# ethz-asl/multipoint

Hardware: AMD Instinct MI355X
Metric: image-pairs/sec (detect+desc+match) @ 480x640 (higher is better)
Workload: dtype f32

## Files before the change

multipoint_amd/build.py:

```python
import concurrent.futures
import os
import subprocess
import sys

HERE = os.path.dirname(os.path.abspath(__file__))
CSRC = os.path.join(HERE, 'csrc')
OBJ_DIR = os.path.join(CSRC, '_build')
LIB_PATH = os.path.join(HERE, 'libmultipoint_hip.so')
SOURCES = ['conv_mfma.hip', 'conv_wino43.hip', 'conv_wino43b.hip', 'conv_split.hip', 'conv_f16.hip', 'conv_f16_res.hip', 'conv_first.hip', 'heads_post.hip', 'head_tail.hip', 'head_tail_f16.hip', 'nms.hip', 'keypoints.hip',
           'sample_desc.hip', 'match_mfma.hip', 'match_guided.hip', 'match_extra.hip', 'pair_metrics.hip', 'detector_metrics.hip', 'homography.hip', 'homography_pooled.hip', 'homog_adapt.hip', 'losses.hip', 'batchnorm_stats.hip', 'photometric.hip', 'shapes.hip', 'api.hip',
           'model_load.hip', 'forward.hip', 'post_api.hip', 'mutual_info.hip', 'align_api.hip', 'pyramid.hip', 'fft.hip', 'lghd.hip', 'lghd_api.hip', 'frames.hip',
           'frames_api.hip', 'draw.hip']
HEADERS = [os.path.join(CSRC, h) for h in ('mp_common.h', 'mp_device.h', 'mp_tile.h', 'mp_f16.h', 'mp_match.h', 'mp_fft.h', 'mp_raster.h', 'mp_homography.h', 'mp_f16_store_pooled.inc',
                                            'mp_f16_store_lines.inc', 'host.h')] + [
    os.path.join(HERE, '..', 'include', 'multipoint_hip.h')]
HIPCC = os.environ.get('HIPCC', '/opt/rocm/bin/hipcc')
FLAGS = ['--offload-arch=gfx950', '-O3', '-std=c++17', '-fPIC', '-Wall', '-Wno-unused-function'] + \
    os.environ.get('MP_HIPCC_FLAGS', '').split()


def _stale(target, deps):
    if not os.path.exists(target):
        return True
    t = os.path.getmtime(target)
    return any(os.path.getmtime(d) > t for d in deps)


DMA_SOURCES = ('conv_wino43.hip', 'conv_wino43b.hip', 'head_tail.hip', 'head_tail_f16.hip')


def check_dma_hazards(asm_path, wait_states=5):
    import re
    lines = open(asm_path).read().split('\n')
    n = 0
    for i, l in enumerate(lines):
        m = re.search(r'global_load_lds_dword(?:x4)? v\d+, s\[(\d+):(\d+)\]', l)
        if not m:
            continue
        n += 1
        base = {int(m.group(1)), int(m.group(2))}
        ws, j = 0, i - 1
        while j >= 0 and ws < wait_states:
            t = lines[j].strip()
            j -= 1
            if t.endswith(':') and not t.startswith(('.Lfunc', ';')) and re.match(r'\.LBB\d+_\d+:', t):
                raise RuntimeError('%s:%d: LDS-DMA only %d wait states behind the branch target %s (needs %d inside the '
                                   'block): open the asm statement with s_nop' % (asm_path, j + 2, ws, t, wait_states))
            if not t or t.startswith((';', '.')) or t.endswith(':'):
                continue
            w = re.match(r'(v_readlane_b32|v_readfirstlane_b32) s(\d+),', t)
            if w and int(w.group(2)) in base:
                raise RuntimeError('%s:%d: %s writes the base SGPR of an LDS-DMA only %d wait states later (needs %d): '
                                   'open the asm statement with s_nop' % (asm_path, j + 2, t, ws, wait_states))
            nop = re.match(r's_nop (\d+)', t)
            ws += int(nop.group(1)) + 1 if nop else 1
    if n == 0:
        raise RuntimeError('%s: no global_load_lds found -- the hazard check is looking at the wrong file' % asm_path)
    return n


SCRATCH_CAPS = {'conv_mfma.hip': 0, 'conv_wino43.hip': 0, 'conv_wino43b.hip': 136, 'conv_split.hip': 0, 'conv_f16.hip': 12,
                'conv_f16_res.hip': 0, 'conv_first.hip': 0, 'head_tail.hip': 0, 'head_tail_f16.hip': 0, 'losses.hip': 0,
                'batchnorm_stats.hip': 0, 'photometric.hip': 0, 'shapes.hip': 0, 'match_mfma.hip': 0, 'match_guided.hip': 0, 'mutual_info.hip': 0, 'pyramid.hip': 0, 'fft.hip': 0, 'lghd.hip': 0,
                'frames.hip': 0, 'draw.hip': 0}


def check_scratch(asm_path, cap):
    import re
    text = open(asm_path).read()
    found = re.findall(r'\.name:\s+(\S+)\n(?:(?!\.name:).*\n)*?\s+\.private_segment_fixed_size:\s+(\d+)', text)
    if not found:
        raise RuntimeError('%s: no kernel metadata found -- the scratch check is looking at the wrong file' % asm_path)
    used = {k: int(v) for k, v in found if int(v) > 0}
    over = {k: v for k, v in used.items() if v > cap}
    if over:
        raise RuntimeError('%s: %d kernel(s) use more scratch than the %d bytes per lane this source is allowed (spilled registers: '
                           'their reloads wait for every load in flight): %s' % (asm_path, len(over), cap, ', '.join(
                               '%s %d B' % (k, v) for k, v in sorted(over.items())[:6])))
    return used


def _compile(src):
    stem = os.path.splitext(src)[0]
    obj = os.path.join(OBJ_DIR, stem + '.o')
    tmp_stem = stem + '.tmp%d' % os.getpid()
    tmp = os.path.join(OBJ_DIR, tmp_stem + '.o')
    extra = ['-save-temps=obj'] if (src in DMA_SOURCES or src in SCRATCH_CAPS) else []
    cmd = [HIPCC] + FLAGS + extra + ['-c', os.path.join(CSRC, src), '-o', tmp]
    try:
        r = subprocess.run(cmd, capture_output=True, text=True)
        if r.returncode != 0:
            raise RuntimeError('hipcc failed for %s:\n%s\n%s' % (src, ' '.join(cmd), r.stderr))
        if src in DMA_SOURCES:
            check_dma_hazards(os.path.join(OBJ_DIR, stem + '-hip-amdgcn-amd-amdhsa-gfx950.s'))
        if src in SCRATCH_CAPS:
            check_scratch(os.path.join(OBJ_DIR, stem + '-hip-amdgcn-amd-amdhsa-gfx950.s'), SCRATCH_CAPS[src])
        os.replace(tmp, obj)
    finally:
        for f in os.listdir(OBJ_DIR):
            if f.startswith(tmp_stem) or f.startswith(stem + '-') or f.startswith(stem + '.hip-'):
                os.remove(os.path.join(OBJ_DIR, f))
    return obj


def build(force=False, verbose=True):
    os.makedirs(OBJ_DIR, exist_ok=True)
    todo = []
    objs = []
    for src in SOURCES:
        obj = os.path.join(OBJ_DIR, os.path.splitext(src)[0] + '.o')
        objs.append(obj)
        if force or _stale(obj, [os.path.join(CSRC, src)] + HEADERS):
            todo.append(src)
    if todo:
        if verbose:
            print('[multipoint_amd.build] hipcc --offload-arch=gfx950: %s' % ', '.join(todo), flush=True)
        with concurrent.futures.ThreadPoolExecutor(max_workers=min(len(todo), os.cpu_count() or 4)) as ex:
            list(ex.map(_compile, todo))
    if force or todo or _stale(LIB_PATH, objs):
        cmd = [HIPCC, '--offload-arch=gfx950', '-shared', '-fPIC', '-o', LIB_PATH] + objs
        r = subprocess.run(cmd, capture_output=True, text=True)
        if r.returncode != 0:
            raise RuntimeError('link failed:\n%s\n%s' % (' '.join(cmd), r.stderr))
        if verbose:
            print('[multipoint_amd.build] linked %s' % LIB_PATH, flush=True)
    return LIB_PATH


if __name__ == '__main__':
    build(force='--force' in sys.argv)
```

multipoint_amd/csrc/conv_wino43.hip:

```cpp
#include "mp_common.h"
#include "mp_device.h"
#include "mp_tile.h"

#include <algorithm>
#include <type_traits>

MP_TIMING_TABLE(g_timing_q, 256 * 8, mp_debug_read_timing_wino43)
MP_TIMING_HEIGHT(g_timing_q_sel, 480, mp_debug_select_height_wino43)

namespace {

constexpr int NPIX = 18 * 34;
constexpr int UC4 = 4;
constexpr int VB4 = UC4 * 32 * 36;
constexpr int UB4 = UC4 * 64 * 36;
constexpr int NRB = (NPIX + 63) / 64;
constexpr int RB4 = NRB * 64 * 4;
constexpr int SW4 = 8 * 36 * 2;


template <int LEAD = 0>
__device__ __forceinline__ void dma16(const float* sbase, unsigned voff_bytes, unsigned lds_byte)
{
    lds_dma<4, LEAD, 0>(sbase, voff_bytes, lds_byte);
}

template <bool POOL, bool BNF, int TC4, bool F1, bool SPLIT = false, bool VIN = false>
__global__ __launch_bounds__(512, 2) void conv_wino43_kernel(const ConvParams p)
{
    static_assert(!(F1 && SPLIT), "the fused first block is never split");
    static_assert(!(VIN && (F1 || SPLIT)), "pre-transformed input: plain launches only");
    constexpr int TR4 = 32 / TC4;
    constexpr int OY = 4 * TR4, OX = 4 * TC4;
    constexpr int PY = OY + 2, PX = OX + 2;
    static_assert(PY * PX == NPIX, "item shape");
    __shared__ __attribute__((aligned(16))) float Vs[(VIN ? 4 : 2) * VB4];
    __shared__ __attribute__((aligned(16))) float Us[2 * UB4];
    __shared__ __attribute__((aligned(16))) float raw[VIN ? 256 : 3 * RB4 + 256];
    __shared__ __attribute__((aligned(16))) float scr[VIN ? 4 : 8 * SW4];
    __shared__ __attribute__((aligned(16))) float prm[(POOL && !SPLIT ? 6 : 3) * 64];

    const int tid = threadIdx.x;
    const int lane = tid & 63;
    const int wave = __builtin_amdgcn_readfirstlane(tid >> 6);
    const int tb = wave & 1, cb = wave >> 1;
    const int NC = SPLIT ? (p.cin / UC4) >> p.ks_shift : p.cin / UC4;

    const XcdRange xr = xcd_range(p.nitems, p.xcd_shift);
    const int stride = xr.stride, item_end = xr.item_end;
    int item = xr.item;
    if (item >= item_end) return;

    struct Where { int slice, img, y0, x0, tile; const float* in_base; };
    auto decode = [&](int it) __attribute__((always_inline)) -> Where {
        Where w{};
        const int tile = (int)udiv((unsigned)it, p.magic_slices, (unsigned)p.nslices);
        w.slice = it - tile * p.nslices;
        w.tile = tile;
        const int trow = (int)udiv((unsigned)tile, p.magic_tx, (unsigned)p.tiles_x);
        const int tx = tile - trow * p.tiles_x;
        const int bi = (int)udiv((unsigned)trow, p.magic_ty, (unsigned)p.tiles_y);
        const int ty = trow - bi * p.tiles_y;
        w.img = p.img_list ? p.img_list[bi] : bi;
        w.y0 = ty * OY; w.x0 = tx * OX;
        w.in_base = p.in_planar ? p.in + (long long)w.img * (p.cin / 4) * p.H * p.W * 4
                                : p.in + (long long)w.img * p.H * p.W * p.in_cstride + p.in_coff;
        if constexpr (SPLIT)
            w.in_base += (long long)((w.slice & ((1 << p.ks_shift) - 1)) * NC) * (p.in_planar ? (long long)p.H * p.W * 4 : UC4);
        return w;
    };

    const int pix_stride = p.in_planar ? 4 : p.in_cstride;
    const long long unit_stride = p.in_planar ? (long long)p.H * p.W * 4 : UC4;
    const int x_shift = p.in_planar == MP_LAYOUT_XPLANAR ? 2 : 0, x_mask = p.in_planar == MP_LAYOUT_XPLANAR ? 3 : 0;
    const int row_stride = p.W * pix_stride;
    auto pixel_off = [&](int y, int x) __attribute__((always_inline)) -> int {
        return y * row_stride + (x >> x_shift) * pix_stride + (x & x_mask) * p.W;
    };
    unsigned rvoff[2];
    bool roff_rel = false;
    auto raw_offsets = [&](const Where& w) __attribute__((always_inline)) -> const float* {
        const bool interior = (w.y0 >= 1) && (w.y0 + OY < p.H) && (w.x0 >= 1) && (w.x0 + OX < p.W);
        if (interior) {
            if (!roff_rel) {
#pragma unroll
                for (int j = 0; j < 2; ++j) {
                    const int f = (wave + 8 * j) * 64 + lane;
                    const int py = f / PX, px = f - py * PX;
                    rvoff[j] = (f < NPIX) ? (unsigned)pixel_off(py, px + x_mask) * 4u : 0u;
                }
                roff_rel = true;
            }
            return w.in_base + pixel_off(w.y0 - 1, w.x0 - 1 - x_mask);
        }
        roff_rel = false;
#pragma unroll
        for (int j = 0; j < 2; ++j) {
            const int f = (wave + 8 * j) * 64 + lane;
            const int py = f / PX, px = f - py * PX;
            unsigned off = 0;
            if (f < NPIX) {
                const int gy = reflect_clamp(w.y0 + py - 1, p.H), gx = reflect_clamp(w.x0 + px - 1, p.W);
                off = (unsigned)pixel_off(gy, gx) * 4u;
            }
            rvoff[j] = off;
        }
        return w.in_base;
    };
    const unsigned raw_lds = lds_addr(raw), us_lds = lds_addr(Us);
    const unsigned raw_m0 = raw_lds + (unsigned)wave * 1024u;
    const unsigned raw_dummy = raw_lds + 3u * RB4 * 4u;
    auto raw_dma = [&](const float* src, unsigned boff_bytes, int j) __attribute__((always_inline)) {
        const unsigned dst = j == 0 ? raw_m0 + boff_bytes : (wave + 8 < NRB ? raw_m0 + 8192u + boff_bytes : raw_dummy);
        dma16(src, rvoff[j], dst);
    };
    const int u_cnt = wave < 4 ? 5 : 4, u_first = wave < 4 ? 5 * wave : 20 + 4 * (wave - 4);
    auto u_dma_site = [&](const float* ub, int buf, int site) __attribute__((always_inline)) {
        if constexpr (VIN) {
#pragma unroll
            for (int i = 3 * site; i < (site ? 5 : 3); ++i) {
                int b = wave + 8 * i;
                b = b < 36 ? b : 35;
                dma16(ub + b * 256, (unsigned)lane * 16u, us_lds + (unsigned)(buf * UB4 + b * 256) * 4u);
            }
            return;
        }
#pragma unroll
        for (int k = 3 * site; k < 3 * site + 3; ++k)
            if (k < u_cnt) {
                const int b = u_first + k;
                dma16<1>(ub + b * 256, (unsigned)lane * 16u, us_lds + (unsigned)(buf * UB4 + b * 256) * 4u);
            }
    };
    auto u_ptr = [&](int slice) __attribute__((always_inline)) -> const float* {
        return p.wpack + (long long)slice * NC * UB4;
    };
    auto load_prm = [&](int vslice) __attribute__((always_inline)) {
        const int slice = SPLIT ? vslice >> p.ks_shift : vslice;
        if (tid < 64) {
            int t = tid;
            if constexpr (F1) asm volatile("" : "+v"(t));
            const float sc = p.scale[slice * 64 + t];
            prm[t] = p.bias[slice * 64 + t]; prm[128 + t] = p.shift[slice * 64 + t];
            if constexpr (POOL && !SPLIT) {
                const bool neg = sc < 0.f;
                prm[64 + t] = fabsf(sc); prm[192 + t] = neg ? -1.f : 1.f;
                prm[256 + t] = __int_as_float(neg ? (int)0x80000000 : 0); prm[320 + t] = __int_as_float(neg ? 0 : 0x7fffffff);
            } else {
                prm[64 + t] = sc;
            }
        }
    };

    const int win = tid >> 3, sub = tid & 7;
    const int w_tile = win >> 1, w_cp = win & 1;
    const int w_ty = w_tile / TC4, w_tx = w_tile % TC4;
    const int sub6 = sub < 6 ? sub : 5;
    const int p1_read = ((4 * w_ty) * PX + 4 * w_tx + sub6) * 4 + 2 * w_cp;
    float* const myscr = scr + wave * SW4 + (win & 7) * 72;
    const unsigned scr_w = lds_addr(myscr + sub6 * 2);
    const int p2_write = (2 * w_cp * 32 + w_tile) * 36 + 6 * sub6;
    f32x2 td[6], tr[6];
    typedef const __attribute__((address_space(3))) f32x2* lds_pair_ptr;
    const unsigned p1_base = lds_addr(raw) + (unsigned)p1_read * 4u;
    unsigned p1_a = p1_base, p1_b = p1_base + 4u * PX * 16u;
    auto tf_pass1 = [&]() __attribute__((always_inline)) {
#pragma unroll
        for (int i = 0; i < 4; ++i) td[i] = reinterpret_cast<lds_pair_ptr>(p1_a)[i * PX * 2];
#pragma unroll
        for (int i = 4; i < 6; ++i) td[i] = reinterpret_cast<lds_pair_ptr>(p1_b)[(i - 4) * PX * 2];
    };
    auto tf_pass1b = [&](unsigned next_byte) __attribute__((always_inline)) {
        bt6(td, tr);
        p1_a = p1_base + next_byte; p1_b = p1_base + 4u * PX * 16u + next_byte;
    };
    auto tf_pass1w = [&](int k) __attribute__((always_inline)) {
        unsigned long long save;
        if (k == 0)
            asm volatile("s_mov_b64 %0, exec\n\ts_and_b64 exec, exec, %4\n\tds_write2_b64 %1, %2, %3 offset0:0 offset1:6\n\ts_mov_b64 exec, %0"
                         : "=&s"(save) : "v"(scr_w), "v"(tr[0]), "v"(tr[1]), "s"(0x3F3F3F3F3F3F3F3Full) : "memory");
        else if (k == 1)
            asm volatile("s_mov_b64 %0, exec\n\ts_and_b64 exec, exec, %4\n\tds_write2_b64 %1, %2, %3 offset0:12 offset1:18\n\ts_mov_b64 exec, %0"
                         : "=&s"(save) : "v"(scr_w), "v"(tr[2]), "v"(tr[3]), "s"(0x3F3F3F3F3F3F3F3Full) : "memory");
        else
            asm volatile("s_mov_b64 %0, exec\n\ts_and_b64 exec, exec, %4\n\tds_write2_b64 %1, %2, %3 offset0:24 offset1:30\n\ts_mov_b64 exec, %0"
                         : "=&s"(save) : "v"(scr_w), "v"(tr[4]), "v"(tr[5]), "s"(0x3F3F3F3F3F3F3F3Full) : "memory");
    };
    auto tf_pass2 = [&]() __attribute__((always_inline)) {
#pragma unroll
        for (int j = 0; j < 6; ++j) td[j] = *reinterpret_cast<const f32x2*>(&myscr[(sub6 * 6 + j) * 2]);
    };
    const unsigned p2_addr = lds_addr(Vs) + (unsigned)p2_write * 4u;
    auto tf_pass2b = [&]() __attribute__((always_inline)) {
        bt6(td, tr);
    };
    auto tf_pass2w = [&](int buf, int k) __attribute__((always_inline)) {
        const unsigned a0 = p2_addr + (unsigned)buf * (VB4 * 4u), a1 = a0 + 32u * 36u * 4u;
        const int j = 2 * k;
        unsigned long long save;
#define MPQ_VST(O0, O1)                                                                                                        \
        asm volatile("s_mov_b64 %0, exec\n\ts_and_b64 exec, exec, %7\n\tds_write2_b32 %1, %2, %3 offset0:" #O0 " offset1:" #O1   \
                     "\n\tds_write2_b32 %4, %5, %6 offset0:" #O0 " offset1:" #O1 "\n\ts_mov_b64 exec, %0"                        \
                     : "=&s"(save) : "v"(a0), "v"(tr[j][0]), "v"(tr[j + 1][0]), "v"(a1), "v"(tr[j][1]), "v"(tr[j + 1][1]),       \
                       "s"(0x3F3F3F3F3F3F3F3Full) : "memory")
        if (k == 0) MPQ_VST(0, 1);
        else if (k == 1) MPQ_VST(2, 3);
        else MPQ_VST(4, 5);
#undef MPQ_VST
    };

    const int a_base = ((lane >> 4) * 64 + cb * 16 + (lane & 15)) * 36;
    const int b_base = ((lane >> 4) * 32 + tb * 16 + (lane & 15)) * 36;
    f32x4 af[3], bf[3];

    constexpr int IW1 = PX + 2, IH1 = PY + 2;
    constexpr int IPB = 768;
    static_assert(!F1 || (IH1 * IW1 <= IPB && 2 * IPB + 16 * 4 + 16 * 48 <= RB4), "F1: patches + parameters + weights must fit the third raw buffer");
    const unsigned ip_lds = raw_lds + 2u * RB4 * 4u;
    const unsigned bst_lds = ip_lds + 2u * IPB * 4u;
    const unsigned w1_lds = bst_lds + 16u * 4u * 4u;
    typedef const __attribute__((address_space(3))) float* lds_f32_ptr;
    typedef const __attribute__((address_space(3))) f32x4* lds_f32x4_ptr;
    typedef __attribute__((address_space(3))) f32x4* lds_f32x4_wptr;
    unsigned pg_x[2] = {0u, 0u}, pg_w[2] = {0u, 0u};
    bool pg_rel = false;
    int pc_par = 0;
    auto prod_offsets = [&](const Where& w) __attribute__((always_inline)) {
        const bool interior = (w.y0 >= 1) && (w.y0 + OY < p.H) && (w.x0 >= 1) && (w.x0 + OX < p.W);
#pragma unroll
        for (int j = 0; j < 2; ++j) {
            const int f = (wave + 8 * j) * 64 + lane;
            const int fc = f < NPIX ? f : NPIX - 1;
            const int py = fc / PX, px = fc - py * PX;
            int oy = py, ox = px;
            if (!interior) {
                oy = reflect_clamp(w.y0 + py - 1, p.H) - w.y0 + 1; ox = reflect_clamp(w.x0 + px - 1, p.W) - w.x0 + 1;
                oy = min(max(oy, 0), IH1 - 3); ox = min(max(ox, 0), IW1 - 3);
            }
            pg_x[j] = ip_lds + (unsigned)(pc_par * IPB + oy * IW1 + ox) * 4u;
            pg_w[j] = (unsigned)f * 16u;
        }
        pg_rel = interior;
    };
    auto patch_dma = [&](const Where& w, int par) __attribute__((always_inline)) {
        const float* const im = p.img + (long long)w.img * p.H * p.W;
#pragma unroll
        for (int j = 0; j < 2; ++j) {
            if (wave * 64 + 512 * j >= IH1 * IW1) continue;
            int q = tid + 512 * j;
            asm volatile("" : "+v"(q));
            q = min(q, IH1 * IW1 - 1);
            const int r = q / IW1, c = q - r * IW1;
            const unsigned off = (unsigned)(reflect_clamp(w.y0 - 2 + r, p.H) * p.W + reflect_clamp(w.x0 - 2 + c, p.W)) * 4u;
            lds_dma<1, 0, 0>(im, off, ip_lds + (unsigned)(par * IPB + wave * 64 + 512 * j) * 4u);
        }
    };
    int pc_unit = 0, pc_next_item = item + stride;
    unsigned pc_wv = w1_lds + (unsigned)min(lane, 47) * 4u;
    unsigned pc_bv = bst_lds;
    float px_[9], qx_[9];
    float pw_;
    f32x4 pd_;
    auto gather_x = [&](float (&x)[9], const int j) __attribute__((always_inline)) {
        const lds_f32_ptr xp = reinterpret_cast<lds_f32_ptr>(pg_x[j]);
#pragma unroll
        for (int t = 0; t < 9; ++t) x[t] = xp[(t / 3) * IW1 + (t % 3)];
    };
    auto tap_mfma = [&](const int t, const float x, const f32x4 c) __attribute__((always_inline)) -> f32x4 {
        switch (t) {
        case 0: return __builtin_amdgcn_mfma_f32_4x4x1f32(pw_, x, c, 4, 0, 0);
        case 1: return __builtin_amdgcn_mfma_f32_4x4x1f32(pw_, x, c, 4, 1, 0);
        case 2: return __builtin_amdgcn_mfma_f32_4x4x1f32(pw_, x, c, 4, 2, 0);
        case 3: return __builtin_amdgcn_mfma_f32_4x4x1f32(pw_, x, c, 4, 3, 0);
        case 4: return __builtin_amdgcn_mfma_f32_4x4x1f32(pw_, x, c, 4, 4, 0);
        case 5: return __builtin_amdgcn_mfma_f32_4x4x1f32(pw_, x, c, 4, 5, 0);
        case 6: return __builtin_amdgcn_mfma_f32_4x4x1f32(pw_, x, c, 4, 6, 0);
        case 7: return __builtin_amdgcn_mfma_f32_4x4x1f32(pw_, x, c, 4, 7, 0);
        default: return __builtin_amdgcn_mfma_f32_4x4x1f32(pw_, x, c, 4, 8, 0);
        }
    };
    auto prod_step = [&](const int k, const unsigned wbuf) __attribute__((always_inline)) {
        if (k == 0) {
            pd_ = reinterpret_cast<lds_f32x4_ptr>(pc_bv)[0];
            pw_ = reinterpret_cast<lds_f32_ptr>(pc_wv)[0];
        } else if (k <= 9) {
            pd_ = tap_mfma(k - 1, px_[k - 1], pd_);
        } else {
            const f32x4 v = {relu_bits(pd_[0]), relu_bits(pd_[1]), relu_bits(pd_[2]), relu_bits(pd_[3])};
            *reinterpret_cast<lds_f32x4_wptr>(raw_lds + wbuf + pg_w[0]) = v;
        }
    };
    auto produce2 = [&](const unsigned wbuf) __attribute__((always_inline)) {
        f32x4 d = tap_mfma(0, qx_[0], pd_);
#pragma unroll
        for (int t = 1; t < 9; ++t) d = tap_mfma(t, qx_[t], d);
        const f32x4 v = {relu_bits(d[0]), relu_bits(d[1]), relu_bits(d[2]), relu_bits(d[3])};
        *reinterpret_cast<lds_f32x4_wptr>(raw_lds + wbuf + pg_w[1]) = v;
    };
    auto produce = [&](const unsigned wbuf) __attribute__((always_inline)) {
        prod_step(0, wbuf);
        if (wave + 8 < NRB) produce2(wbuf);
#pragma unroll
        for (int k = 1; k <= 10; ++k) prod_step(k, wbuf);
    };
    auto prod_advance = [&]() __attribute__((always_inline)) {
        pc_wv += 48u * 4u; pc_bv += 4u * 4u;
        if (++pc_unit == NC) {
            pc_unit = 0;
            pc_wv -= (unsigned)NC * 48u * 4u; pc_bv -= (unsigned)NC * 4u * 4u;
            if (pc_next_item < item_end) {
                const Where w = decode(pc_next_item);
                pc_par ^= 1;
                if (!(pg_rel && (w.y0 >= 1) && (w.y0 + OY < p.H) && (w.x0 >= 1) && (w.x0 + OX < p.W))) prod_offsets(w);
                else {
                    const unsigned flip = pc_par ? (unsigned)IPB * 4u : 0u - (unsigned)IPB * 4u;
                    pg_x[0] += flip; pg_x[1] += flip;
                }
                gather_x(px_, 0);
                if (wave + 8 < NRB) gather_x(qx_, 1);
                pc_next_item += stride;
            }
        }
    };

    const unsigned vs_lds = lds_addr(Vs);
    auto v_dma = [&](const float* vsrc, int slot, int i) __attribute__((always_inline)) {
        const int b = wave + 8 * i;
        const unsigned dst = b < 18 ? vs_lds + (unsigned)(slot * VB4 + b * 256) * 4u : lds_addr(raw);
        dma16(vsrc + (b < 18 ? b : 17) * 256, (unsigned)lane * 16u, dst);
    };
    const float* vcur = nullptr;
    int v_chunk = 0, v_next_item = item + stride;
    auto v_advance = [&]() __attribute__((always_inline)) {
        vcur += VB4;
        if (++v_chunk == NC) {
            v_chunk = 0;
            if (v_next_item < item_end) {
                vcur = p.vglobal + (long long)decode(v_next_item).tile * NC * VB4;
                v_next_item += stride;
            } else {
                vcur -= (long long)NC * VB4;
            }
        }
    };

    Where cur = decode(item);
    if constexpr (F1) {
        for (int f = tid; f < 16 * 48; f += 512) {
            const int u = f / 48, l = f - u * 48;
            (raw + 2 * RB4 + 2 * IPB + 16 * 4)[f] = l < 36 ? p.w1[(l >> 2) * 64 + 4 * u + (l & 3)] : 0.f;
        }
        if (tid < 64) (raw + 2 * RB4 + 2 * IPB)[tid] = p.b1[tid];
        patch_dma(cur, 0);
        if (item + stride < item_end) patch_dma(decode(item + stride), 1);
        prod_offsets(cur);
        dma_wait();
        __syncthreads();
        gather_x(px_, 0);
        if (wave + 8 < NRB) gather_x(qx_, 1);
        produce(0u);
        prod_advance();
        produce(RB4 * 4u);
        prod_advance();
    }
    const float* rbase = (F1 || VIN) ? p.in : raw_offsets(cur);
    const float* rsrc = rbase;
    Where ld_item = cur;
    int ld_chunk = 0;
    int ld_next_item = item + stride;
    auto ld_advance = [&]() __attribute__((always_inline)) {
        rsrc += unit_stride;
        if (++ld_chunk == NC) {
            ld_chunk = 0;
            if (ld_next_item < item_end) {
                ld_item = decode(ld_next_item);
                rbase = raw_offsets(ld_item);
                ld_next_item += stride;
            }
            rsrc = rbase;
        }
    };
    const float* up = u_ptr(cur.slice);
    if constexpr (VIN) {
        vcur = p.vglobal + (long long)cur.tile * NC * VB4;
#pragma unroll
        for (int u = 0; u < 3; ++u) {
            v_dma(vcur, u, 0); v_dma(vcur, u, 1); v_dma(vcur, u, 2);
            v_advance();
        }
    } else if constexpr (!F1) {
        raw_dma(rsrc, 0u, 0); raw_dma(rsrc, 0u, 1); ld_advance();
        raw_dma(rsrc, RB4 * 4u, 0); raw_dma(rsrc, RB4 * 4u, 1); ld_advance();
        raw_dma(rsrc, 2u * RB4 * 4u, 0); raw_dma(rsrc, 2u * RB4 * 4u, 1); ld_advance();
    }
    unsigned rd_byte = 0u, rt_byte = RB4 * 4u;
    u_dma_site(up, 0, 0); u_dma_site(up, 0, 1);
    u_dma_site(up + UB4, 1, 0); u_dma_site(up + UB4, 1, 1);
    load_prm(cur.slice);
    dma_wait();
    __syncthreads();
    if constexpr (!VIN) {
        tf_pass1(); tf_pass1b(RB4 * 4u); tf_pass1w(0); tf_pass1w(1); tf_pass1w(2); tf_pass2(); tf_pass2b();
        tf_pass2w(0, 0); tf_pass2w(0, 1); tf_pass2w(0, 2);
        asm volatile("s_waitcnt lgkmcnt(0)" ::: "memory");
        __syncthreads();
    }
    af[0] = *reinterpret_cast<const f32x4*>(&Us[a_base]);
    bf[0] = *reinterpret_cast<const f32x4*>(&Vs[b_base]);
    af[1] = *reinterpret_cast<const f32x4*>(&Us[a_base + 4]);
    bf[1] = *reinterpret_cast<const f32x4*>(&Vs[b_base + 4]);

    const f32x4 zero4 = {0.f, 0.f, 0.f, 0.f};
    int cur_par = 0;
#ifdef MP_TIMING
    unsigned long long tsum[8] = {0, 0, 0, 0, 0, 0, 0, 0};
    const bool t_on = ((POOL ? p.H : -p.H) == g_timing_q_sel);
#endif
    for (;;) {
        MP_CLOCK(t_item);
        f32x4 acc[36];
        const int item_next = item + stride;
        const bool has_next = item_next < item_end;
        const int next_slice = has_next ? (int)(item_next - (int)udiv((unsigned)item_next, p.magic_slices, (unsigned)p.nslices) * p.nslices)
                                        : cur.slice;
        const float* unext = u_ptr(next_slice);
        auto tf_at = [&](const int g, const int e, const int vb) __attribute__((always_inline)) {
            constexpr int S[2][8][2] = {
                {{0, 2}, {2, 2}, {2, 3}, {3, 1}, {3, 2}, {5, 2}, {5, 3}, {6, 1}},
                {{0, 2}, {2, 2}, {2, 3}, {3, 1}, {3, 2}, {4, 3}, {5, 1}, {6, 1}}};
            constexpr int TFS = (TC4 == 8 && !F1) ? 1 : 0;
            auto at = [&](const int k) { return g == S[TFS][k][0] && e == S[TFS][k][1]; };
            if (at(0)) tf_pass1();
            if (at(1)) { tf_pass1b(F1 ? (unsigned)vb * (RB4 * 4u) : 3u * RB4 * 4u - rd_byte - rt_byte); tf_pass1w(0); }
            if (at(2)) tf_pass1w(1);
            if (at(3)) tf_pass1w(2);
            if (at(4)) tf_pass2();
            if (at(5)) { tf_pass2b(); tf_pass2w(vb ^ 1, 0); }
            if (at(6)) tf_pass2w(vb ^ 1, 1);
            if (at(7)) tf_pass2w(vb ^ 1, 2);
        };
        auto prod_at = [&](const int g, const int e, const int vb) __attribute__((always_inline)) {
            const unsigned wbuf = (unsigned)vb * (RB4 * 4u);
            constexpr int slot_g[11] = {0, 0, 1, 1, 1, 2, 3, 4, 4, 4, 5};
            constexpr int slot_e[11] = {0, 3, 1, 2, 3, 1, 3, 1, 2, 3, 1};
#pragma unroll
            for (int k = 0; k <= 10; ++k)
                if (g == slot_g[k] && e == slot_e[k]) prod_step(k, wbuf);
            if (g == 0 && e == 0) { if (wave + 8 < NRB) produce2(wbuf); }
        };
        auto unit_body = [&](const int c, auto first_tag, auto vb_tag, auto vs_tag) __attribute__((always_inline)) {
            constexpr bool FIRST = decltype(first_tag)::value;
            constexpr int vb = decltype(vb_tag)::value;
            constexpr int vs = VIN ? decltype(vs_tag)::value : vb;
            constexpr int vsn = VIN ? (vs + 1) & 3 : vb ^ 1;
            const float* const ur = Us + vb * UB4 + a_base;
            const float* const vr = Vs + vs * VB4 + b_base;
            const float* const urn = Us + (vb ^ 1) * UB4 + a_base;
            const float* const vrn = Vs + vsn * VB4 + b_base;
            const float* const un2 = c + 2 < NC ? up + (long long)(c + 2) * UB4 : unext + (long long)(c + 2 - NC) * UB4;
            MP_CLOCK(t_u0);
#ifdef MP_TIMING
            unsigned long long t_b0 = 0, t_b1 = 0;
#endif
#pragma unroll
            for (int g = 0; g < 9; ++g) {
#pragma unroll
                for (int e = 0; e < 4; ++e) {
                    const int s = 4 * g + e;
                    acc[s] = __builtin_amdgcn_mfma_f32_16x16x4f32(af[g % 3][e], bf[g % 3][e], FIRST ? zero4 : acc[s], 0, 0, 0);
                    __builtin_amdgcn_sched_barrier(0);
                    if constexpr (!VIN) { if (e != 2) tf_at(g, e, vb); }
                    if constexpr (F1) prod_at(g, e, vb);
                    if (e == 0) {
                        af[(g + 2) % 3] = *reinterpret_cast<const f32x4*>(g + 2 < 9 ? &ur[4 * (g + 2)] : &urn[4 * (g - 7)]);
                        bf[(g + 2) % 3] = *reinterpret_cast<const f32x4*>(g + 2 < 9 ? &vr[4 * (g + 2)] : &vrn[4 * (g - 7)]);
                    } else if (e == 1) {
                        if (g == 7) u_dma_site(un2, vb, 0);
                        else if (g == 8) u_dma_site(un2, vb, 1);
                        else if (g == 0) { if constexpr (VIN) v_dma(vcur, (vs + 3) & 3, 0); else if constexpr (!F1) raw_dma(rsrc, rd_byte, 0); }
                        else if (g == 1) { if constexpr (VIN) v_dma(vcur, (vs + 3) & 3, 1); else if constexpr (!F1) raw_dma(rsrc, rd_byte, 1); }
                        else if (g == 2) { if constexpr (VIN) v_dma(vcur, (vs + 3) & 3, 2); }
                    } else if (e == 2) {
                        if constexpr (!VIN) tf_at(g, 2, vb);
                    } else {
                        if (g == 6) {
#ifdef MP_TIMING
                            t_b0 = __builtin_amdgcn_s_memtime();
#endif
                            if constexpr (F1) asm volatile("s_waitcnt vmcnt(0) lgkmcnt(0)" ::: "memory");
                            else if constexpr (VIN) asm volatile("s_waitcnt vmcnt(3) lgkmcnt(0)" ::: "memory");
                            else asm volatile("s_waitcnt vmcnt(2) lgkmcnt(0)" ::: "memory");
#ifdef MP_TIMING
                            t_b1 = __builtin_amdgcn_s_memtime();
#endif
                            __syncthreads();
#ifdef MP_TIMING
                            tsum[4] += __builtin_amdgcn_s_memtime() - t_b1;
#endif
                        }
                    }
                    __builtin_amdgcn_sched_barrier(0);
                }
            }
            MP_CLOCK(t_u1);
            MP_CLOCK_ADD(0, t_u0, t_u1);
            MP_CLOCK_ADD(1, t_b0, t_b1);
        };
        auto unit = [&](const int c, auto first_tag, auto vb_tag, auto vs_tag) __attribute__((always_inline)) {
            unit_body(c, first_tag, vb_tag, vs_tag);
            if constexpr (VIN) {
                v_advance();
            } else if constexpr (F1) {
                prod_advance();
            } else {
                ld_advance();
                const unsigned ro = 3u * RB4 * 4u - rd_byte - rt_byte;
                rd_byte = rt_byte; rt_byte = ro;
            }
        };
        using VB0 = std::integral_constant<int, 0>;
        using VB1 = std::integral_constant<int, 1>;
        using VS2 = std::integral_constant<int, 2>;
        using VS3 = std::integral_constant<int, 3>;
        if constexpr (VIN) {
            unit(0, std::true_type{}, VB0{}, VB0{});
            for (int c = 1; c + 3 < NC; c += 4) {
                unit(c, std::false_type{}, VB1{}, VB1{});
                unit(c + 1, std::false_type{}, VB0{}, VS2{});
                unit(c + 2, std::false_type{}, VB1{}, VS3{});
                unit(c + 3, std::false_type{}, VB0{}, VB0{});
            }
            unit(NC - 3, std::false_type{}, VB1{}, VB1{});
            unit(NC - 2, std::false_type{}, VB0{}, VS2{});
            unit(NC - 1, std::false_type{}, VB1{}, VS3{});
        } else {
        unit(0, std::true_type{}, VB0{}, VB0{});
        for (int c = 1; c + 1 < NC; c += 2) {
            unit(c, std::false_type{}, VB1{}, VB1{});
            unit(c + 1, std::false_type{}, VB0{}, VB0{});
        }
        unit(NC - 1, std::false_type{}, VB1{}, VB1{});
        }

        MP_CLOCK(t_e0);
        MP_CLOCK_ADD(3, t_item, t_e0);
        if constexpr (F1) { if (item_next + stride < item_end) patch_dma(decode(item_next + stride), cur_par); }
        const int tl = tb * 16 + (lane & 15);
        const int cl = cb * 16 + 4 * (lane >> 4);
        const f32x4 b4 = *reinterpret_cast<const f32x4*>(&prm[cl]);
        const f32x4 s4 = *reinterpret_cast<const f32x4*>(&prm[64 + cl]);
        const f32x4 t4 = *reinterpret_cast<const f32x4*>(&prm[128 + cl]);
        const int oy = cur.y0 + 4 * (tl / TC4), ox = cur.x0 + 4 * (tl % TC4);
        const int ch0 = (SPLIT ? cur.slice >> p.ks_shift : cur.slice) * 64 + cl;
        const int cs = p.out_cstride;
        constexpr int NO = POOL ? 2 : 4;
        f32x2 keep[NO][NO];
        if constexpr (SPLIT) {
            unsigned long long* const part = reinterpret_cast<unsigned long long*>(p.split_scratch) + (long long)item * (2 * 16 * 512) + tid;
#pragma unroll
            for (int h = 0; h < 2; ++h) {
                f32x2 tcol[4][6];
#pragma unroll
                for (int j = 0; j < 6; ++j) {
                    f32x2 m[6], y[4];
#pragma unroll
                    for (int i = 0; i < 6; ++i) m[i] = f32x2{acc[6 * i + j][2 * h], acc[6 * i + j][2 * h + 1]};
                    at6s(m, y);
#pragma unroll
                    for (int a = 0; a < 4; ++a) tcol[a][j] = y[a];
                }
#pragma unroll
                for (int a = 0; a < 4; ++a) {
                    f32x2 y[4];
                    at6s(tcol[a], y);
#pragma unroll
                    for (int b = 0; b < 4; ++b)
                        part[(h * 16 + a * 4 + b) * 512] = __builtin_bit_cast(unsigned long long, y[b]);
                }
            }
        }
        if constexpr (!SPLIT) {
#pragma unroll
        for (int h = 0; h < 2; ++h) {
            f32x2 tcol[4][6];
            if constexpr (!SPLIT) {
#pragma unroll
            for (int j = 0; j < 6; ++j) {
                f32x2 m[6], y[4];
#pragma unroll
                for (int i = 0; i < 6; ++i) m[i] = f32x2{acc[6 * i + j][2 * h], acc[6 * i + j][2 * h + 1]};
                at6s(m, y);
#pragma unroll
                for (int a = 0; a < 4; ++a) tcol[a][j] = y[a];
            }
            }
            const f32x2 bb = {b4[2 * h], b4[2 * h + 1]}, ss = {s4[2 * h], s4[2 * h + 1]}, tt = {t4[2 * h], t4[2 * h + 1]};
            f32x2 res[NO][NO];
            if constexpr (POOL) {
                const f32x4 g4 = *reinterpret_cast<const f32x4*>(&prm[192 + cl]);
                const f32x4 lo4 = *reinterpret_cast<const f32x4*>(&prm[256 + cl]), hi4 = *reinterpret_cast<const f32x4*>(&prm[320 + cl]);
                const f32x2 gg = {g4[2 * h], g4[2 * h + 1]};
                const f32x2 gb = bb * gg;
                constexpr float A1 = (float)MP_W43_A, A2 = A1 * A1, A3 = A2 * A1, A4 = A2 * A2;
                const f32x2 gk[5] = {gg, gg * f32x2{A1, A1}, gg * f32x2{A2, A2}, gg * f32x2{A3, A3}, gg * f32x2{A4, A4}};
                f32x2 xv[4][4];
#pragma unroll
                for (int a = 0; a < 4; ++a) {
                    f32x2 y[4];
                    at6s(tcol[a], y);
#pragma unroll
                    for (int b = 0; b < 4; ++b) {
                        const int e = (a == 1 ? 1 : a == 2 ? 2 : 0) + (b == 1 ? 1 : b == 2 ? 2 : 0);
                        xv[a][b] = __builtin_elementwise_fma(y[b], gk[e], gb);
                    }
                }
#pragma unroll
                for (int a = 0; a < NO; ++a)
#pragma unroll
                    for (int b = 0; b < NO; ++b) {
                        f32x2 m;
#pragma unroll
                        for (int r = 0; r < 2; ++r)
                            m[r] = fmaxf(fmaxf(xv[2 * a][2 * b][r], xv[2 * a][2 * b + 1][r]), fmaxf(xv[2 * a + 1][2 * b][r], xv[2 * a + 1][2 * b + 1][r]));
                        if (BNF) {
                            m = __builtin_elementwise_fma(m, ss, tt);
                            m = f32x2{relu_bits(m[0]), relu_bits(m[1])};
                        } else {
#pragma unroll
                            for (int r = 0; r < 2; ++r)
                                asm("v_med3_i32 %0, %1, %2, %3" : "=v"(m[r]) : "v"(m[r]), "v"(lo4[2 * h + r]), "v"(hi4[2 * h + r]));
                            m = __builtin_elementwise_fma(m, ss, tt);
                        }
                        res[a][b] = m;
                    }
            } else {
            f32x2 yv[4][4];
#pragma unroll
            for (int a = 0; a < 4; ++a) {
                f32x2 y[4];
                at6s(tcol[a], y);
#pragma unroll
                for (int b = 0; b < 4; ++b) {
                    f32x2 v = w43_add_bias(y[b], a, b, bb);
                    if (BNF) { v = v * ss + tt; v = f32x2{relu_bits(v[0]), relu_bits(v[1])}; }
                    else { v = f32x2{relu_bits(v[0]), relu_bits(v[1])}; v = v * ss + tt; }
                    yv[a][b] = v;
                }
            }
#pragma unroll
            for (int a = 0; a < NO; ++a)
#pragma unroll
                for (int b = 0; b < NO; ++b) res[a][b] = yv[a][b];
            }
            if (h == 0) {
#pragma unroll
                for (int a = 0; a < NO; ++a)
#pragma unroll
                    for (int b = 0; b < NO; ++b) keep[a][b] = res[a][b];
            } else {
                const int Ho = POOL ? p.H >> 1 : p.H, Wo = POOL ? p.W >> 1 : p.W;
                const int py0 = POOL ? oy >> 1 : oy, px0 = POOL ? ox >> 1 : ox;
                const bool xpl = !POOL && p.out_planar == MP_LAYOUT_XPLANAR;
                char* const img_base = reinterpret_cast<char*>(
                    p.out_planar ? p.out + (long long)cur.img * (p.cout / 4) * Ho * Wo * 4
                                 : p.out + (long long)cur.img * Ho * Wo * cs + p.out_coff);
                const unsigned ps = xpl ? (unsigned)Wo * 4u : p.out_planar ? 16u : (unsigned)cs * 4u;
                const unsigned rs = p.out_planar ? (unsigned)Wo * 16u : (unsigned)Wo * ps;
                const unsigned o0 = xpl ? (unsigned)(((ch0 >> 2) * Ho + py0) * Wo * 4 + px0) * 4u
                                  : p.out_planar ? (unsigned)(((ch0 >> 2) * Ho + py0) * Wo + px0) * 16u
                                                 : (unsigned)((py0 * Wo + px0) * cs + ch0) * 4u;
                if (oy < p.H && ox < p.W && ch0 < p.cout) {
#pragma unroll
                    for (int a = 0; a < NO; ++a)
#pragma unroll
                        for (int b = 0; b < NO; ++b) {
                            const f32x4 v = {keep[a][b][0], keep[a][b][1], res[a][b][0], res[a][b][1]};
                            *reinterpret_cast<f32x4*>(img_base + (o0 + (unsigned)a * rs + (unsigned)b * ps)) = v;
                        }
                }
            }
        }
        }
        MP_CLOCK(t_e1);
        MP_CLOCK_ADD(2, t_e0, t_e1);
#ifdef MP_TIMING
        tsum[7] += 1;
        if (!has_next && tid == 0 && t_on)
            for (int i = 0; i < 8; ++i) g_timing_q[blockIdx.x * 8 + i] = tsum[i];
#endif
        if (!has_next) { dma_wait(); return; }
        if (next_slice != cur.slice) {
            __syncthreads();
            load_prm(next_slice);
        }
        item = item_next;
        cur = decode(item);
        cur_par ^= 1;
        up = unext;
    }
}

template <int TC4>
__global__ __launch_bounds__(256) void wino43_vprod_kernel(const ConvParams p, long long ntb)
{
    constexpr int TR4 = 32 / TC4, OY = 4 * TR4, OX = 4 * TC4;
    __shared__ __attribute__((aligned(16))) float st[19456];
    const int ncp = p.cin >> 1, NC = p.cin / UC4;
    const int TL = 256 / ncp;
    const int RS = TL * 36 + 4;
    const int groups = 32 / TL;
    const int tid = threadIdx.x;
    const int cp = tid % ncp, tlc = tid / ncp;
    const long long tb = (long long)blockIdx.x / groups;
    const int t0 = ((int)((long long)blockIdx.x % groups)) * TL, t = t0 + tlc;
    (void)ntb;
    const int tx = (int)(tb % p.tiles_x);
    const long long trow = tb / p.tiles_x;
    const int ty = (int)(trow % p.tiles_y);
    const int bi = (int)(trow / p.tiles_y);
    const int img = p.img_list ? p.img_list[bi] : bi;
    const int wy = ty * OY + 4 * (t / TC4) - 1, wx = tx * OX + 4 * (t % TC4) - 1;
    const float* const base = p.in + (long long)img * p.H * p.W * p.in_cstride + p.in_coff + 2 * cp;
    int gx[6];
#pragma unroll
    for (int j = 0; j < 6; ++j) gx[j] = reflect_clamp(wx + j, p.W);
    f32x2 r[6][6];
#pragma unroll
    for (int j = 0; j < 6; ++j) {
        f32x2 d[6], o[6];
#pragma unroll
        for (int i = 0; i < 6; ++i)
            d[i] = *reinterpret_cast<const f32x2*>(base + ((long long)reflect_clamp(wy + i, p.H) * p.W + gx[j]) * p.in_cstride);
        bt6(d, o);
#pragma unroll
        for (int i = 0; i < 6; ++i) r[i][j] = o[i];
    }
    float* const dst0 = st + (2 * cp) * RS + tlc * 36;
    float* const dst1 = dst0 + RS;
#pragma unroll
    for (int i = 0; i < 6; i += 2) {
        f32x2 a[6], b[6];
        bt6(r[i], a);
        bt6(r[i + 1], b);
        *reinterpret_cast<f32x4*>(dst0 + 6 * i) = f32x4{a[0][0], a[1][0], a[2][0], a[3][0]};
        *reinterpret_cast<f32x4*>(dst0 + 6 * i + 4) = f32x4{a[4][0], a[5][0], b[0][0], b[1][0]};
        *reinterpret_cast<f32x4*>(dst0 + 6 * i + 8) = f32x4{b[2][0], b[3][0], b[4][0], b[5][0]};
        *reinterpret_cast<f32x4*>(dst1 + 6 * i) = f32x4{a[0][1], a[1][1], a[2][1], a[3][1]};
        *reinterpret_cast<f32x4*>(dst1 + 6 * i + 4) = f32x4{a[4][1], a[5][1], b[0][1], b[1][1]};
        *reinterpret_cast<f32x4*>(dst1 + 6 * i + 8) = f32x4{b[2][1], b[3][1], b[4][1], b[5][1]};
    }
    __syncthreads();
    const int q4 = TL * 9, total4 = p.cin * q4;
    float* const gbase = p.vglobal + (tb * NC * 4 * 32 + t0) * 36;
    for (int i = tid; i < total4; i += 256) {
        const int row = i / q4, w = i - row * q4;
        *reinterpret_cast<f32x4*>(gbase + (long long)row * (32 * 36) + w * 4) = *reinterpret_cast<const f32x4*>(st + row * RS + w * 4);
    }
}

template <bool POOL, int TC4, bool F1 = false, bool SPLIT = false>
int launch_q(const ConvParams& p, hipStream_t s)
{
    constexpr int OY = 4 * (32 / TC4), OX = 4 * TC4;
    ConvParams q = p;
    if (SPLIT) q.nslices = p.nslices << p.ks_shift;
    q.tiles_x = (p.W + OX - 1) / OX; q.tiles_y = (p.H + OY - 1) / OY;
    const long long nitems = (long long)p.B * q.tiles_x * q.tiles_y * q.nslices;
    if (nitems <= 0) return 0;
    if (tile_items(q, nitems)) return 1;
    const unsigned grid = persistent_grid(nitems, p.ncu, p.xcd_shift);
    const ConvParams& pp = q;
    if (p.bn_first) hipLaunchKernelGGL((conv_wino43_kernel<POOL, true, TC4, F1, SPLIT>), dim3(grid), dim3(512), 0, s, pp);
    else hipLaunchKernelGGL((conv_wino43_kernel<POOL, false, TC4, F1, SPLIT>), dim3(grid), dim3(512), 0, s, pp);
    return 0;
}

template <int TC4>
int launch_vin(const ConvParams& p, hipStream_t s)
{
    constexpr int OY = 4 * (32 / TC4), OX = 4 * TC4;
    ConvParams q = p;
    q.tiles_x = (p.W + OX - 1) / OX; q.tiles_y = (p.H + OY - 1) / OY;
    const long long ntb = (long long)p.B * q.tiles_x * q.tiles_y, nitems = ntb * q.nslices;
    if (nitems <= 0) return 0;
    if (tile_items(q, nitems)) return 1;
    const ConvParams& pp = q;
    const int tl = 256 / (p.cin / 2);
    hipLaunchKernelGGL((wino43_vprod_kernel<TC4>), dim3((unsigned)(ntb * (32 / tl))), dim3(256), 0, s, pp, ntb);
    const unsigned grid = persistent_grid(nitems, p.ncu, p.xcd_shift);
    if (p.bn_first) hipLaunchKernelGGL((conv_wino43_kernel<false, true, TC4, false, false, true>), dim3(grid), dim3(512), 0, s, pp);
    else hipLaunchKernelGGL((conv_wino43_kernel<false, false, TC4, false, false, true>), dim3(grid), dim3(512), 0, s, pp);
    return 0;
}

template <bool POOL, bool SPLIT = false>
int launch_shape(const ConvParams& p, hipStream_t s)
{
    const long long wide = (long long)((p.W + 31) / 32) * ((p.H + 15) / 16), tall = (long long)((p.W + 15) / 16) * ((p.H + 31) / 32);
    return tall < wide ? launch_q<POOL, 4, false, SPLIT>(p, s) : launch_q<POOL, 8, false, SPLIT>(p, s);
}

}

bool conv_wino43_supports(const ConvParams& p)
{
    return !p.pad_zero && p.cin % 8 == 0 && p.cout % 4 == 0 && p.H % 4 == 0 && p.W % 4 == 0 && p.H >= 4 && p.W >= 4 &&
           p.in_cstride % 4 == 0 && p.in_coff % 4 == 0 && p.out_cstride % 4 == 0 && p.out_coff % 4 == 0;
}

long long conv_wino43_vglobal_floats(const ConvParams& p)
{
    const long long wide = (long long)((p.W + 31) / 32) * ((p.H + 15) / 16), tall = (long long)((p.W + 15) / 16) * ((p.H + 31) / 32);
    return (long long)p.B * std::min(wide, tall) * (p.cin / UC4) * VB4;
}

long long conv_wino43_items(const ConvParams& p)
{
    const long long wide = (long long)((p.W + 31) / 32) * ((p.H + 15) / 16), tall = (long long)((p.W + 15) / 16) * ((p.H + 31) / 32);
    return (long long)p.B * std::min(wide, tall) * p.nslices;
}

int launch_conv_wino43(const ConvParams& p, bool pool, hipStream_t s, bool fuse_first)
{
    if (p.out_planar == MP_LAYOUT_XPLANAR && pool) return 2;
    if ((p.in_planar == MP_LAYOUT_XPLANAR || p.out_planar == MP_LAYOUT_XPLANAR) && p.ks_shift > 0) return 2;
    if (fuse_first) return pool && p.cin == 64 ? launch_q<true, 8, true>(p, s) : 2;
    if (p.vglobal) {
        if (pool || p.ks_shift > 0 || p.cin % 16 != 0 || p.in_planar || p.cin > 256 || 256 % (p.cin / 2) != 0 || (p.cin / 2) < 8) return 2;
        const long long wide = (long long)((p.W + 31) / 32) * ((p.H + 15) / 16), tall = (long long)((p.W + 15) / 16) * ((p.H + 31) / 32);
        return tall < wide ? launch_vin<4>(p, s) : launch_vin<8>(p, s);
    }
    if (p.ks_shift > 0) {
        const int ncs = (p.cin / 4) >> p.ks_shift;
        if (ncs < 4 || (ncs & 1) || (ncs << p.ks_shift) * 4 != p.cin || !p.split_scratch) return 2;
        const int rc = pool ? launch_shape<true, true>(p, s) : launch_shape<false, true>(p, s);
        return rc ? rc : launch_split_reduce(p, 1, pool, s);
    }
    return pool ? launch_shape<true>(p, s) : launch_shape<false>(p, s);
}
```

Before: 3508.

## Skip dummy raw DMAs per wave and rebalance weight DMA sites with scalar-branch asm

Waves with no second raw block now skip the LDS-DMA entirely via an inline-asm scalar branch, instead of issuing a dummy load into a padding region. The padding is dropped from the raw buffer for non-F1 variants. The per-wave U-weight DMA split is reassigned, in the non-F1, non-VIN case, so the fifth load lands on waves that skip the raw load. The barrier wait becomes wave-dependent to match the changed vmcnt counts. The build-time hazard checker learns to walk past the new skip labels, at the cost of more fragile hand-written asm and vmcnt bookkeeping.

```diff
diff --git a/multipoint_amd/build.py b/multipoint_amd/build.py
--- a/multipoint_amd/build.py
+++ b/multipoint_amd/build.py
@@ -46,6 +46,17 @@
             if t.endswith(':') and not t.startswith(('.Lfunc', ';')) and re.match(r'\.LBB\d+_\d+:', t):
                 raise RuntimeError('%s:%d: LDS-DMA only %d wait states behind the branch target %s (needs %d inside the '
                                    'block): open the asm statement with s_nop' % (asm_path, j + 2, ws, t, wait_states))
+            skip = re.match(r'(\.Lmp_skip_\d+):', t)
+            if skip:
+                k = j
+                while k >= 0 and not re.match(r's_cbranch_scc[01] %s$' % re.escape(skip.group(1)), lines[k].strip()):
+                    if re.match(r'\.LBB\d+_\d+:', lines[k].strip()) or j - k > 16:
+                        k = -1
+                    k -= 1
+                if k < 0:
+                    raise RuntimeError('%s:%d: no s_cbranch_scc to %s in its own asm statement' % (asm_path, j + 2, skip.group(1)))
+                j = k
+                continue
             if not t or t.startswith((';', '.')) or t.endswith(':'):
                 continue
             w = re.match(r'(v_readlane_b32|v_readfirstlane_b32) s(\d+),', t)
diff --git a/multipoint_amd/csrc/conv_wino43.hip b/multipoint_amd/csrc/conv_wino43.hip
--- a/multipoint_amd/csrc/conv_wino43.hip
+++ b/multipoint_amd/csrc/conv_wino43.hip
@@ -23,6 +23,21 @@
 __device__ __forceinline__ void dma16(const float* sbase, unsigned voff_bytes, unsigned lds_byte)
 {
     lds_dma<4, LEAD, 0>(sbase, voff_bytes, lds_byte);
+}
+
+template <unsigned MASK>
+__device__ __forceinline__ void dma16_waves(int wave, const float* sbase, unsigned voff_bytes, unsigned lds_byte)
+{
+    unsigned keep;
+    asm volatile("s_bitcmp1_b32 %5, %4\n\ts_cbranch_scc0 .Lmp_skip_%=\n\ts_mov_b32 %0, m0\n\ts_mov_b32 m0, %3\n\ts_nop 2\n\t"
+                 "global_load_lds_dwordx4 %1, %2\n\ts_mov_b32 m0, %0\n.Lmp_skip_%=:"
+                 : "=&s"(keep) : "v"(voff_bytes), "s"(sbase), "s"(lds_byte), "s"(wave), "n"(MASK) : "memory", "scc");
+}
+template <unsigned MASK>
+__device__ __forceinline__ void dma_wait_waves_2(int wave)
+{
+    asm volatile("s_waitcnt vmcnt(2) lgkmcnt(0)\n\ts_bitcmp1_b32 %1, %0\n\ts_cbranch_scc1 .Lmp_skip_%=\n\ts_waitcnt vmcnt(1)\n.Lmp_skip_%=:"
+                 :: "s"(wave), "n"(MASK) : "memory", "scc");
 }
 
 template <bool POOL, bool BNF, int TC4, bool F1, bool SPLIT = false, bool VIN = false>
@@ -36,7 +51,7 @@
     static_assert(PY * PX == NPIX, "item shape");
     __shared__ __attribute__((aligned(16))) float Vs[(VIN ? 4 : 2) * VB4];
     __shared__ __attribute__((aligned(16))) float Us[2 * UB4];
-    __shared__ __attribute__((aligned(16))) float raw[VIN ? 256 : 3 * RB4 + 256];
+    __shared__ __attribute__((aligned(16))) float raw[VIN ? 256 : F1 ? 3 * RB4 + 256 : 3 * RB4];
     __shared__ __attribute__((aligned(16))) float scr[VIN ? 4 : 8 * SW4];
     __shared__ __attribute__((aligned(16))) float prm[(POOL && !SPLIT ? 6 : 3) * 64];
 
@@ -109,12 +124,15 @@
     };
     const unsigned raw_lds = lds_addr(raw), us_lds = lds_addr(Us);
     const unsigned raw_m0 = raw_lds + (unsigned)wave * 1024u;
-    const unsigned raw_dummy = raw_lds + 3u * RB4 * 4u;
+    constexpr unsigned RAW2 = (1u << (NRB - 8)) - 1u;
     auto raw_dma = [&](const float* src, unsigned boff_bytes, int j) __attribute__((always_inline)) {
-        const unsigned dst = j == 0 ? raw_m0 + boff_bytes : (wave + 8 < NRB ? raw_m0 + 8192u + boff_bytes : raw_dummy);
-        dma16(src, rvoff[j], dst);
-    };
-    const int u_cnt = wave < 4 ? 5 : 4, u_first = wave < 4 ? 5 * wave : 20 + 4 * (wave - 4);
+        if (j == 0) dma16(src, rvoff[0], raw_m0 + boff_bytes);
+        else dma16_waves<RAW2>(wave, src, rvoff[1], raw_m0 + 8192u + boff_bytes);
+    };
+    constexpr bool EVEN = !F1 && !VIN;
+    constexpr unsigned U5 = 0x3cu;
+    const int u_cnt = EVEN ? ((U5 >> wave) & 1 ? 5 : 4) : wave < 4 ? 5 : 4;
+    const int u_first = EVEN ? (wave < 2 ? 4 * wave : wave < 6 ? 5 * wave - 2 : 4 * wave + 4) : wave < 4 ? 5 * wave : 20 + 4 * (wave - 4);
     auto u_dma_site = [&](const float* ub, int buf, int site) __attribute__((always_inline)) {
         if constexpr (VIN) {
 #pragma unroll
@@ -122,6 +140,15 @@
                 int b = wave + 8 * i;
                 b = b < 36 ? b : 35;
                 dma16(ub + b * 256, (unsigned)lane * 16u, us_lds + (unsigned)(buf * UB4 + b * 256) * 4u);
+            }
+            return;
+        }
+        if constexpr (EVEN) {
+#pragma unroll
+            for (int k = 3 * site; k < 3 * site + 3 && k < 5; ++k) {
+                const int b = u_first + k;
+                if (k < 4) dma16(ub + b * 256, (unsigned)lane * 16u, us_lds + (unsigned)(buf * UB4 + b * 256) * 4u);
+                else dma16_waves<U5>(wave, ub + b * 256, (unsigned)lane * 16u, us_lds + (unsigned)(buf * UB4 + b * 256) * 4u);
             }
             return;
         }
@@ -489,7 +516,7 @@
 #endif
                             if constexpr (F1) asm volatile("s_waitcnt vmcnt(0) lgkmcnt(0)" ::: "memory");
                             else if constexpr (VIN) asm volatile("s_waitcnt vmcnt(3) lgkmcnt(0)" ::: "memory");
-                            else asm volatile("s_waitcnt vmcnt(2) lgkmcnt(0)" ::: "memory");
+                            else dma_wait_waves_2<RAW2>(wave);
 #ifdef MP_TIMING
                             t_b1 = __builtin_amdgcn_s_memtime();
 #endif
```

Result: no change. 3519, median of 6 (+0.3%).
